# lonelycorn/mvSLAM

Hardware: AMD Instinct MI355X
Metric: image-pairs/sec (2k kp, 50k RANSAC hyp) (higher is better)
Workload: dtype f64; 1 GPU; 512 independent synthetic 640x480 pairs per GPU, 2000 keypoints (256-bit descriptors), 50000 8-point hypotheses per pair, full match+RANSAC+decompose+triangulate; pairs_per_gpu=512, keypoints=2000, hypotheses=50000, parallelism=pairs sharded, dp1, streams=2

## Files before the change

mvslam_amd/csrc/kernels.hip:

```cpp
#include <algorithm>
#include "kernels.hpp"

#include "device_math.hpp"
#include "match_fp4.hpp"
#include "prescreen.hpp"

namespace mvs {

constexpr uint32_t kKeyNone = 0xffffffffu;
__device__ __forceinline__ uint32_t bcnt_acc(uint32_t x, uint32_t acc)
{
    uint32_t r;
    asm("v_bcnt_u32_b32 %0, %1, %2" : "=v"(r) : "v"(x), "v"(acc));
    return r;
}
__device__ __forceinline__ void key_insert(uint32_t &k0, uint32_t &k1, uint32_t k)
{
    uint32_t m;
    asm("v_med3_u32 %0, %1, %2, %3" : "=v"(m) : "v"(k0), "v"(k1), "v"(k));
    k1 = m;
    k0 = min(k0, k);
}

constexpr int kTopkWaves = 16;
// ... 2425 lines not shown
                best = s_cnt[c];
                win = c;
            }
        s_win = win;
    }
    __syncthreads();
    const int win = s_win;
    if (win < 0) {
        clear_tail(0);
        return;
    }
    const double *src = b.cand_pts + ((size_t)pair * 4 + win) * b.max_kp * 3;
    const uint8_t *okw = okf + (size_t)win * b.max_kp;
    const uint16_t *inl = b.inl + base;
    const int n_pts = block_compact(
        n_inl, s_tot, [&](int j) { return okw[j] != 0; },
        [&](int j, int pos) {
            double *d = b.points + (base + pos) * 3;
            d[0] = src[j * 3]; d[1] = src[j * 3 + 1]; d[2] = src[j * 3 + 2];
            b.point_idx[base + pos] = inl[j];
        });
    clear_tail(n_pts);
    if (tid == 0) {
        const double *Rw = fm->R[win >> 1];
        const bool flip = (win & 1) != 0;
        const double t[3] = {flip ? -fm->T[0] : fm->T[0], flip ? -fm->T[1] : fm->T[1], flip ? -fm->T[2] : fm->T[2]};
        double Rr[3][3], RT[3][3];
#pragma unroll
        for (int i = 0; i < 3; ++i)
#pragma unroll
            for (int j = 0; j < 3; ++j) {
                Rr[i][j] = Rw[i * 3 + j];
                res->R1to2[i * 3 + j] = Rw[i * 3 + j];
            }
        rectify3(Rr);
#pragma unroll
        for (int i = 0; i < 3; ++i)
#pragma unroll
            for (int j = 0; j < 3; ++j)
                RT[i][j] = Rr[j][i];
        rectify3(RT);
#pragma unroll
        for (int i = 0; i < 3; ++i) {
            res->t1to2[i] = t[i];
            res->t[i] = -((RT[i][0] * t[0] + RT[i][1] * t[1]) + RT[i][2] * t[2]);
#pragma unroll
            for (int j = 0; j < 3; ++j)
                res->R[i * 3 + j] = RT[i][j];
        }
        res->n_points = n_pts;
        res->valid = 1;
    }
}

#ifdef MVS_DEBUG_HOOKS
#include "kernels_experiments.hip"
#endif

constexpr int kCntThreads = 768;
constexpr int kCntPpl = 2;
constexpr int kSolveBlock = 64;
#ifdef MVS_DEBUG_HOOKS
static int kSplitMinPairs = 3;
void set_split_min_pairs(int v) { kSplitMinPairs = v; }
#else
constexpr int kSplitMinPairs = 3;
#endif

static bool prescreened_launch(const BatchDev &b, int n_active, int H)
{
    const int cus = b.cu_count > 0 ? b.cu_count : 256;
    return n_active >= kSplitMinPairs || (kSplitMinPairs == 3 && n_active == 2 && 2 * ((H + kHypPerBlock - 1) / kHypPerBlock) > cus);
}

static size_t count_lds_bytes(int max_kp)
{
    const int bw = 64 * kCntPpl;
    return (size_t)((max_kp + bw - 1) / bw) * bw * 4 * sizeof(double);
}

bool kernel_desc(int id, int max_kp, int desc_words, KernelDesc *out)
{
    KernelDesc d{nullptr, nullptr, 0, 0};
    switch (id) {
    case kKMatchTopk:
        d.name = desc_words == 4 ? "match_topk_kernel<4>" : desc_words == 16 ? "match_topk_kernel<16>" : "match_mfma_kernel<true>";
        d.fn = desc_words == 4    ? reinterpret_cast<const void *>(match_topk_kernel<4>)
               : desc_words == 16 ? reinterpret_cast<const void *>(match_topk_kernel<16>)
                                  : reinterpret_cast<const void *>(match_mfma_kernel<true>);
        d.threads = desc_words == 8 ? kMmThreads : 1024;
        break;
    case kKMatchTopkVec:
        d.name = "match_topk_kernel<8>";
        d.fn = reinterpret_cast<const void *>(match_topk_kernel<8>);
        d.threads = 1024;
        break;
    case kKMatchCompact:
        d.name = "match_compact_kernel";
        d.fn = reinterpret_cast<const void *>(match_compact_kernel);
        d.threads = 1024;
        break;
    case kKRansacFused:
        d.name = "ransac_kernel<false, true, (mvs::Solve)2>";
        d.fn = reinterpret_cast<const void *>(ransac_kernel<false, true, Solve::GuardedCheap>);
        d.threads = kHypPerBlock;
        break;
    case kKRansacSolve:
        d.name = "ransac_solve_list_kernel";
        d.fn = reinterpret_cast<const void *>(ransac_solve_list_kernel);
        d.threads = kSolveBlock;
        break;
    case kKRansacSelect:
        d.name = "ransac_select_kernel";
        d.fn = reinterpret_cast<const void *>(ransac_select_kernel);
        d.threads = kSelThreads;
        d.dynamic_lds = (size_t)max_kp * 4 * sizeof(double);
        break;
    case kKPairPrepare:
        d.name = "pair_prepare_kernel";
        d.fn = reinterpret_cast<const void *>(pair_prepare_kernel);
        d.threads = 256;
        break;
    case kKRansacPrescreen:
        d.name = "ransac_prescreen_kernel";
        d.fn = reinterpret_cast<const void *>(ransac_prescreen_kernel);
        d.threads = 64;
        break;
    case kKRansacExactList:
        d.name = "ransac_exact_list_kernel";
        d.fn = reinterpret_cast<const void *>(ransac_exact_list_kernel);
        d.threads = 64;
        break;
    case kKRansacCount2:
        d.name = "ransac_count2_kernel<768, 2>";
        d.fn = reinterpret_cast<const void *>(ransac_count2_kernel<kCntThreads, kCntPpl>);
        d.threads = kCntThreads;
        d.dynamic_lds = count_lds_bytes(max_kp);
        break;
    case kKRansacCountPilot:
        d.name = "ransac_finish_mfma_kernel<false, true>";
        d.fn = reinterpret_cast<const void *>(ransac_finish_mfma_kernel<false, true>);
        d.threads = kFinishThreads;
        d.dynamic_lds = (size_t)kDenseChunk * 64;
        break;
    case kKRansacCountFinish:
        d.name = "ransac_finish_mfma_kernel<false, false>";
        d.fn = reinterpret_cast<const void *>(ransac_finish_mfma_kernel<false>);
        d.threads = kFinishThreads;
        d.dynamic_lds = (size_t)kDenseChunk * 64;
        break;
    case kKRansacCountFinishRest:
        d.name = "ransac_finish_upper_kernel<false>";
        d.fn = reinterpret_cast<const void *>(ransac_finish_upper_kernel<false>);
        d.threads = kFinUpperThreads;
        d.dynamic_lds = (size_t)kFinUpperChunk * 64 + (size_t)(kFinUpperThreads / 64) * kDenseWin * 16;
        break;
    case kKRansacCountMfma:
        d.name = "ransac_count_mfma_kernel<false, 512, 4, 672>";
        d.fn = reinterpret_cast<const void *>(ransac_count_mfma_kernel<false, kDenseThreads, kDenseBatches>);
        d.threads = kDenseThreads;
        d.dynamic_lds = (size_t)kDenseChunkD * 64 + (size_t)(kDenseThreads / 64) * kDenseWin * 16;
        break;
    case kKRansacSurvivors:
        d.name = "ransac_survivors_kernel";
        d.fn = reinterpret_cast<const void *>(ransac_survivors_kernel);
        d.threads = 256;
        break;
    case kKFinModel:
        d.name = "finalize_model_kernel";
        d.fn = reinterpret_cast<const void *>(finalize_model_kernel);
        d.threads = kFinThreads;
        break;
    case kKTriangulate:
        d.name = "triangulate_kernel";
        d.fn = reinterpret_cast<const void *>(triangulate_kernel);
        d.threads = 256;
        break;
    case kKFinSelect:
        d.name = "finalize_select_kernel";
        d.fn = reinterpret_cast<const void *>(finalize_select_kernel);
        d.threads = kFinThreads;
        break;
#ifdef MVS_DEBUG_HOOKS
    case kKRansacCount32:
        d.name = "ransac_count32_kernel<768, 4, 4, 1, false>";
        d.fn = reinterpret_cast<const void *>(ransac_count32_kernel<kCnt32Threads, kCnt32Ppl, kCnt32Slots, 1>);
        d.threads = kCnt32Threads;
        d.dynamic_lds = count32_lds_bytes(max_kp);
        break;
#endif
    default: return false;
    }
    *out = d;
    return true;
}

hipError_t prepare_kernels()
{
    const void *fns[] = {
#ifdef MVS_DEBUG_HOOKS
                         reinterpret_cast<const void *>(ransac_count32_kernel<kCnt32Threads, kCnt32Ppl, kCnt32Slots, 1>),
                         reinterpret_cast<const void *>(ransac_count32_kernel<kCnt32Threads, kCnt32Ppl, kCnt32Slots, 1, true>),
                         reinterpret_cast<const void *>(ransac_count32_kernel<kCnt32Threads, kCnt32Ppl, kCnt32Slots, 2>),
                         reinterpret_cast<const void *>(ransac_count32_kernel<kCnt32Threads, kCnt32Ppl, kCnt32Slots, 2, true>),
#endif
                         reinterpret_cast<const void *>(ransac_count2_kernel<kCntThreads, kCntPpl>),
                         reinterpret_cast<const void *>(ransac_count2_kernel<kCntThreads, kCntPpl, true>),
                         reinterpret_cast<const void *>(ransac_count_mfma_kernel<false, kDenseThreads, kDenseBatches>),
                         reinterpret_cast<const void *>(ransac_count_mfma_kernel<true, kDenseThreads, kDenseBatches>),
                         reinterpret_cast<const void *>(ransac_finish_mfma_kernel<false>),
                         reinterpret_cast<const void *>(ransac_finish_mfma_kernel<true>),
                         reinterpret_cast<const void *>(ransac_finish_mfma_kernel<false, true>),
                         reinterpret_cast<const void *>(ransac_finish_mfma_kernel<true, true>),
                         reinterpret_cast<const void *>(ransac_finish_upper_kernel<false>),
                         reinterpret_cast<const void *>(ransac_finish_upper_kernel<true>),
                         reinterpret_cast<const void *>(ransac_select_kernel)};
    for (const void *f : fns) {
        const hipError_t e = hipFuncSetAttribute(f, hipFuncAttributeMaxDynamicSharedMemorySize, kMaxKp * 32);
        if (e != hipSuccess)
            return e;
    }
    return hipSuccess;
}

#ifdef MVS_DEBUG_HOOKS
static int g_match_mfma = 1;
void set_match_mfma(int v) { g_match_mfma = v; }
#else
constexpr int g_match_mfma = 1;
#endif

void launch_match_topk(const BatchDev &b, const RunParams &rp, int n_active, hipStream_t stream, LaunchTimer *lt)
{
    const dim3 grid((b.max_kp + 63) / 64, n_active), block(1024);
    const double ratio = rp.ratio, md = rp.max_dist;
    const int mm_groups8 = ((b.max_kp + kMmQueries - 1) / kMmQueries) * n_active;
    const bool mfma8 = b.desc_words == 8 && (g_match_mfma == 2 || (g_match_mfma == 1 && mm_groups8 >= 512));
    if (lt) lt->mark(b.desc_words == 8 && !mfma8 ? kKMatchTopkVec : kKMatchTopk);
    switch (b.desc_words) {
    case 4: hipLaunchKernelGGL(match_topk_kernel<4>, grid, block, 0, stream, b, ratio, md); break;
    case 8: {
        if (mfma8) {
            const dim3 mgrid((b.max_kp + kMmQueries - 1) / kMmQueries, n_active);
            const int cap = match_cap_distance(ratio, md);
            if (cap >= 0)
                hipLaunchKernelGGL(match_mfma_kernel<true>, mgrid, dim3(kMmThreads), 0, stream, b, ratio, md, cap);
            else
                hipLaunchKernelGGL(match_mfma_kernel<false>, mgrid, dim3(kMmThreads), 0, stream, b, ratio, md, 0);
        } else
            hipLaunchKernelGGL(match_topk_kernel<8>, grid, block, 0, stream, b, ratio, md);
        break;
    }
    case 16: hipLaunchKernelGGL(match_topk_kernel<16>, grid, block, 0, stream, b, ratio, md); break;
    default: break;
    }
}

void launch_match_compact(const BatchDev &b, const RunParams &, int n_active, hipStream_t stream, LaunchTimer *lt)
{
    if (lt) lt->mark(kKMatchCompact);
    hipLaunchKernelGGL(match_compact_kernel, dim3(n_active), dim3(1024), 0, stream, b);
}

void launch_prep_points(const BatchDev &b, const double *uv1, const double *uv2, int n_active, hipStream_t stream)
{
    hipLaunchKernelGGL(prep_points_kernel, dim3((b.max_kp + 255) / 256, n_active), dim3(256), 0, stream, b, uv1, uv2);
}

#ifdef MVS_DEBUG_HOOKS
static int g_count_dense = 1;
static int g_dense_margin = kDenseMargin;
static int g_pilot_hyp = kPilotMfmaHyp;
void set_count_dense(int v)
{
    if (v >= 100000)
        g_pilot_hyp = v - 100000;
    else if (v >= 1000)
        g_dense_margin = v - 1000;
    else
        g_count_dense = v;
}
static int g_force_mode = -1;
void set_prescreen_force(int m) { g_force_mode = m; }
hipError_t prescreen_fallback_waves(unsigned int *out, bool reset)
{
    hipError_t e = hipMemcpyFromSymbol(out, HIP_SYMBOL(g_ps_fallback_waves), sizeof(*out));
    const unsigned int zero = 0;
    if (e == hipSuccess && reset)
        e = hipMemcpyToSymbol(HIP_SYMBOL(g_ps_fallback_waves), &zero, sizeof(zero));
    return e;
}

void launch_prescreen_only(const BatchDev &b, const RunParams &rp, int n_active, int mode, hipStream_t stream)
{
    hipLaunchKernelGGL(pair_prepare_kernel, dim3(n_active), dim3(256), 0, stream, b, rp, mode);
    hipLaunchKernelGGL(ransac_prescreen_kernel, dim3((rp.num_hypotheses + 63) / 64, n_active), dim3(64), 0, stream, b, rp);
}
#else
constexpr int g_dense_margin = kDenseMargin;
constexpr int g_pilot_hyp = kPilotMfmaHyp;
constexpr int g_force_mode = -1;
#endif

static void launch_counting(const BatchDev &b, const RunParams &rp, int n_active, hipStream_t stream, LaunchTimer *lt, bool stats,
                            hipEvent_t after_dense = nullptr)
{
    const int H = rp.num_hypotheses;
    const int n_groups4 = (H + kCntSlots - 1) / kCntSlots;
    const int wpw = kCntThreads / 64;
    int wg = (512 + n_active - 1) / n_active;
    wg = std::max(wg, 4);
    wg = std::min(wg, std::max(1, (n_groups4 + wpw - 1) / wpw));
    const size_t lds_cnt = count_lds_bytes(b.max_kp);
#ifdef MVS_DEBUG_HOOKS
    if (g_count_dense == 0) {
        if (lt) lt->mark(kKRansacCount32);
        launch_count32<1>(b, rp, wg, n_active, stats, stream);
    } else
#endif
    {
        if (lt) lt->mark(kKRansacCountPilot);
        const dim3 pilot_grid(n_active, (std::min(H, g_pilot_hyp) + kFinishThreads - 1) / kFinishThreads);
        if (stats)
            hipLaunchKernelGGL((ransac_finish_mfma_kernel<true, true>), pilot_grid, dim3(kFinishThreads), (size_t)kDenseChunk * 64,
                               stream, b, rp, 0);
        else
            hipLaunchKernelGGL((ransac_finish_mfma_kernel<false, true>), pilot_grid, dim3(kFinishThreads), (size_t)kDenseChunk * 64,
                               stream, b, rp, 0);
        if (lt) lt->mark(kKRansacCountMfma);
        const size_t lds_dense = (size_t)kDenseChunkD * 64 + (size_t)(kDenseThreads / 64) * kDenseWin * 16;
        const dim3 dense_grid(((H + kDenseThreads - 1) / kDenseThreads + kDenseBatches - 1) / kDenseBatches, n_active);
        if (stats)
            hipLaunchKernelGGL((ransac_count_mfma_kernel<true, kDenseThreads, kDenseBatches>), dense_grid, dim3(kDenseThreads),
                               lds_dense, stream, b, rp, g_dense_margin);
        else
            hipLaunchKernelGGL((ransac_count_mfma_kernel<false, kDenseThreads, kDenseBatches>), dense_grid, dim3(kDenseThreads),
                               lds_dense, stream, b, rp, g_dense_margin);
        if (after_dense) (void)hipEventRecord(after_dense, stream);
        if (lt) lt->mark(kKRansacCountFinish);
#ifdef MVS_DEBUG_HOOKS
        if (g_count_dense == 2) {
            launch_count32<2>(b, rp, wg, n_active, stats, stream);
        } else
#endif
        {
            hipLaunchKernelGGL(ransac_list_sort_kernel, dim3(n_active), dim3(kSortThreads), 0, stream, b);
            if (stats)
                hipLaunchKernelGGL(ransac_finish_mfma_kernel<true>, dim3(n_active, 1), dim3(kFinishThreads), (size_t)kDenseChunk * 64,
                                   stream, b, rp, 0);
            else
                hipLaunchKernelGGL(ransac_finish_mfma_kernel<false>, dim3(n_active, 1), dim3(kFinishThreads), (size_t)kDenseChunk * 64,
                                   stream, b, rp, 0);
            if ((H + kFinishThreads - 1) / kFinishThreads > 1) {
                const size_t lds_up = (size_t)kFinUpperChunk * 64 + (size_t)(kFinUpperThreads / 64) * kDenseWin * 16;
                if (lt) lt->mark(kKRansacCountFinishRest);
                if (stats)
                    hipLaunchKernelGGL(ransac_finish_upper_kernel<true>, dim3(n_active, kFinUpperWg), dim3(kFinUpperThreads), lds_up,
                                       stream, b, rp);
                else
                    hipLaunchKernelGGL(ransac_finish_upper_kernel<false>, dim3(n_active, kFinUpperWg), dim3(kFinUpperThreads), lds_up,
                                       stream, b, rp);
            }
        }
    }
    if (lt) lt->mark(kKRansacCount2);
    if (stats)
        hipLaunchKernelGGL((ransac_count2_kernel<kCntThreads, kCntPpl, true>), dim3(wg, n_active), dim3(kCntThreads), lds_cnt,
                           stream, b, rp, wg);
    else
        hipLaunchKernelGGL((ransac_count2_kernel<kCntThreads, kCntPpl>), dim3(wg, n_active), dim3(kCntThreads), lds_cnt, stream,
                           b, rp, wg);
}

static void launch_prescreened(const BatchDev &b, const RunParams &rp, int n_active, hipStream_t stream, LaunchTimer *lt,
                               bool stats, hipEvent_t after_dense = nullptr)
{
    const int H = rp.num_hypotheses;
    const int G = (H + kHypPerBlock - 1) / kHypPerBlock;
    if (lt) lt->mark(kKPairPrepare);
    hipLaunchKernelGGL(pair_prepare_kernel, dim3(n_active), dim3(256), 0, stream, b, rp, g_force_mode);
    if (lt) lt->mark(kKRansacPrescreen);
    hipLaunchKernelGGL(ransac_prescreen_kernel, dim3((H + 63) / 64, n_active), dim3(64), 0, stream, b, rp);
    if (lt) lt->mark(kKRansacSolve);
    hipLaunchKernelGGL(mode0_list_kernel, dim3(1), dim3(256), 0, stream, b, n_active);
    static_assert(kSolveBlock == 64, "ransac_solve_list_kernel takes blocks of 64 hypotheses");
    hipLaunchKernelGGL(ransac_solve_list_kernel, dim3(2048), dim3(64), 0, stream, b, rp,
                       G * (kHypPerBlock / kSolveBlock));
    launch_counting(b, rp, n_active, stream, lt, stats, after_dense);
    if (lt) lt->mark(kKRansacSurvivors);
    hipLaunchKernelGGL(ransac_survivors_kernel, dim3(kSurvWg, n_active), dim3(256), 0, stream, b, rp, n_active);
    if (lt) lt->mark(kKRansacExactList);
    hipLaunchKernelGGL(ransac_exact_list_kernel, dim3(1024), dim3(64), 0, stream, b, rp, 0);
    if (lt) lt->mark(kKRansacSelect);
    hipLaunchKernelGGL(ransac_select_kernel, dim3(n_active), dim3(kSelThreads), (size_t)b.max_kp * 4 * sizeof(double), stream,
                       b, rp, 1);
}

void launch_ransac(const BatchDev &b, const RunParams &rp, int n_active, bool stats, hipStream_t stream, LaunchTimer *lt,
                   hipEvent_t after_dense)
{
    const int G = (rp.num_hypotheses + kHypPerBlock - 1) / kHypPerBlock;
    const dim3 grid(G, n_active), block(kHypPerBlock);
    const bool split_ok = !stats && b.hyp_F && prescreened_launch(b, n_active, rp.num_hypotheses);
    if (!split_ok || b.hyp_count) {
        if (lt) lt->mark(kKRansacFused);
        if (!stats)
            hipLaunchKernelGGL((ransac_kernel<false, true, Solve::GuardedCheap>), grid, block, 0, stream, b, rp);
        else
            hipLaunchKernelGGL((ransac_kernel<true, true, Solve::Guarded>), grid, block, 0, stream, b, rp);
        if (stats && b.hyp_F && !b.hyp_count && prescreened_launch(b, n_active, rp.num_hypotheses))
            launch_prescreened(b, rp, n_active, stream, nullptr, true);
    } else {
        launch_prescreened(b, rp, n_active, stream, lt, false, after_dense);
    }
}

void launch_finalize(const BatchDev &b, const RunParams &rp, int n_active, int mode, hipStream_t stream, LaunchTimer *lt)
{
    if (lt) lt->mark(kKFinModel);
    hipLaunchKernelGGL(finalize_model_kernel, dim3(n_active), dim3(kFinThreads), 0, stream, b, rp, mode);
    if (lt) lt->mark(kKTriangulate);
    hipLaunchKernelGGL(triangulate_kernel, dim3((b.max_kp + 255) / 256, n_active), dim3(256), 0, stream, b);
    if (lt) lt->mark(kKFinSelect);
    hipLaunchKernelGGL(finalize_select_kernel, dim3(n_active), dim3(kFinThreads), 0, stream, b);
}

#ifdef MVS_DEBUG_HOOKS
#include "kernels_audit.hip"
#endif


__global__ __launch_bounds__(256) void single_params_kernel(BatchDev b, SingleParams sp, const uint4 *in)
{
    const int t = blockIdx.x * 256 + threadIdx.x;
    if (t == 0) {
        const_cast<int32_t *>(b.n1)[0] = sp.n1;
        const_cast<int32_t *>(b.n2)[0] = sp.n2;
        const_cast<int64_t *>(b.gidx)[0] = sp.gidx;
    }
    if (t < 9) {
        const_cast<double *>(b.K)[t] = sp.K[t];
        const_cast<double *>(b.Kinv)[t] = sp.Kinv[t];
    }
    if (in) {
        uint4 *dst[4] = {reinterpret_cast<uint4 *>(const_cast<uint32_t *>(b.desc1)), reinterpret_cast<uint4 *>(const_cast<uint32_t *>(b.desc2)),
                         reinterpret_cast<uint4 *>(const_cast<float *>(b.kp1)), reinterpret_cast<uint4 *>(const_cast<float *>(b.kp2))};
        size_t off = 0;
#pragma unroll
        for (int k = 0; k < 4; ++k) {
            const size_t n16 = sp.part_bytes[k] / 16;
            for (size_t i = t; i < n16; i += (size_t)gridDim.x * 256)
                dst[k][i] = in[off + i];
            if (t == 0 && (sp.part_bytes[k] & 8u))
                reinterpret_cast<uint2 *>(dst[k] + n16)[0] = reinterpret_cast<const uint2 *>(in + off + n16)[0];
            off += (sp.part_bytes[k] + 15) / 16;
        }
    }
}
void launch_single_params(const BatchDev &b, const SingleParams &sp, const void *in, hipStream_t stream)
{
    hipLaunchKernelGGL(single_params_kernel, dim3(in ? 32 : 1), dim3(256), 0, stream, b, sp, reinterpret_cast<const uint4 *>(in));
}
__global__ __launch_bounds__(256) void single_gather_kernel(BatchDev b, int rows, int flags, unsigned char *out)
{
    const SingleLayout L = single_layout(rows, flags);
    const int tid = blockIdx.x * 256 + threadIdx.x, nth = gridDim.x * 256;
    const uint32_t *r32 = reinterpret_cast<const uint32_t *>(b.results);
    for (int i = tid; i < (int)(sizeof(mvs_pair_result) / 4); i += nth)
        reinterpret_cast<uint32_t *>(out)[i] = r32[i];
    if (flags & 1)
        for (int i = tid; i < rows; i += nth)
            out[L.mask + i] = b.mask[i];
    if (flags & 2)
        for (int i = tid; i < rows * 3; i += nth)
            reinterpret_cast<double *>(out + L.points)[i] = b.points[i];
    if (flags & 4)
        for (int i = tid; i < rows; i += nth)
            reinterpret_cast<int32_t *>(out + L.idx)[i] = b.point_idx[i];
    if (flags & 8)
        for (int i = tid; i < rows; i += nth)
            reinterpret_cast<mvs_match *>(out + L.matches)[i] = b.matches[i];
}
void launch_single_gather(const BatchDev &b, int rows, int flags, unsigned char *out, hipStream_t stream)
{
    hipLaunchKernelGGL(single_gather_kernel, dim3(16), dim3(256), 0, stream, b, rows, flags, out);
}

void launch_fundamental(const double *p1, const double *p2, double *F, int *ok, hipStream_t stream)
{
    hipLaunchKernelGGL(fundamental_kernel, dim3(1), dim3(64), 0, stream, p1, p2, F, ok);
}

}
```

mvslam_amd/csrc/kernels_audit.hip:

```cpp
#ifndef MVS_DEBUG_HOOKS
#error "kernels_audit.hip belongs to the diagnostics build"
#endif

__global__ __launch_bounds__(256) void pairstep_check_kernel(const double *rows, int n, unsigned long long *out)
{
    const int i = blockIdx.x * 256 + threadIdx.x;
    if (i >= n)
        return;
    double A[2][2][3], V[2][2][3], W[2][2];
#pragma unroll
    for (int v = 0; v < 2; ++v) {
#pragma unroll
        for (int r = 0; r < 2; ++r) {
            double sd = 0.0;
#pragma unroll
            for (int k = 0; k < 3; ++k) {
                A[v][r][k] = rows[(size_t)i * 6 + r * 3 + k];
                V[v][r][k] = r == k ? 1.0 : 0.0;
                sd = dfma(A[v][r][k], A[v][r][k], sd);
            }
            W[v][r] = sd;
        }
    }
    {
        const double g2 = dfma(W[0][0], W[0][0], W[0][1] * W[0][1]) + 0x1p-300;
        double h;
        const double gamma = sqrt_fast_nz_h(g2, h);
        const double e = dabs(dfma(-gamma, h + h, 1.0));
        atomicMax(&out[3], (unsigned long long)__double_as_longlong(e));
    }
    bool ch0 = false, ch1 = false, bad0 = false, bad1 = false;
    unsigned r0 = 0, r1 = 0;
    double q0 = 0x1p1000, q1 = 0x1p1000;
    jacobi_pair<3, 3, true, true, true>(A[0][0], A[0][1], V[0][0], V[0][1], W[0][0], W[0][1], ch0, r0, bad0, q0);
    jacobi_pair<3, 3, false, false, false>(A[1][0], A[1][1], V[1][0], V[1][1], W[1][0], W[1][1], ch1, r1, bad1, q1);
    if (ch0 != ch1) {
        atomicAdd(&out[2], 1ull);
        return;
    }
    if (!ch0 || !(q0 >= kGuardQMin) || !(W[1][0] + W[1][1] <= kGuardWSumMax))
        return;
    atomicAdd(&out[1], 1ull);
    bool same = __double_as_longlong(W[0][0]) == __double_as_longlong(W[1][0]) &&
                __double_as_longlong(W[0][1]) == __double_as_longlong(W[1][1]);
#pragma unroll
    for (int r = 0; r < 2; ++r)
#pragma unroll
        for (int k = 0; k < 3; ++k)
            same = same && __double_as_longlong(A[0][r][k]) == __double_as_longlong(A[1][r][k]) &&
                   __double_as_longlong(V[0][r][k]) == __double_as_longlong(V[1][r][k]);
    if (!same)
        atomicAdd(&out[0], 1ull);
}

void launch_pairstep_check(const double *rows, int n, unsigned long long *out, hipStream_t stream)
{
    hipLaunchKernelGGL(pairstep_check_kernel, dim3((n + 255) / 256), dim3(256), 0, stream, rows, n, out);
}

void launch_fastmath_check(const double *x, const double *y, int n, unsigned long long *out, hipStream_t stream)
{
    hipLaunchKernelGGL(fastmath_check_kernel, dim3((n + 255) / 256), dim3(256), 0, stream, x, y, n, out);
}


template <int PHASE>
__global__ __launch_bounds__(256, 1) void audit_kernel(BatchDev b, RunParams rp, unsigned long long *out, int32_t *maxc)
{
    extern __shared__ __attribute__((aligned(16))) double s_apts[];
    const int pair = blockIdx.y, g = blockIdx.x, tid = threadIdx.x, lane = tid & 63;
    const int M = min(b.M[pair], b.max_kp);
    if (M < 8)
        return;
    const int H = rp.num_hypotheses;
    const uint32_t h = (uint32_t)g * kHypPerBlock + tid;
    const bool live = h < (uint32_t)H;
    const uint32_t hh = live ? h : (uint32_t)(H - 1);
    const uint64_t seed = rp.seed + (uint64_t)b.gidx[pair];
    const double *P = b.pts + (size_t)pair * b.max_kp * 4;
    {
        const double2 *src = reinterpret_cast<const double2 *>(P);
        double2 *dst = reinterpret_cast<double2 *>(s_apts);
        for (int i = tid; i < 2 * M; i += kHypPerBlock)
            dst[i] = src[i];
        __syncthreads();
    }
    double F[9];
    unsigned rot = 0, pairs = 0;
    bool bad = false;
    bool ok = solve_hypothesis<Solve::GuardedCheap>(seed, hh, M, rp.sampler, P, F, rot, pairs, bad);
    if (__builtin_expect(__any(bad), 0)) {
        rot = 0;
        pairs = 0;
        ok = solve_hypothesis<Solve::Ieee>(seed, hh, M, rp.sampler, P, F, rot, pairs, bad);
    }
    const unsigned sweeps = pairs / 36u;
    const double thr = pair_max_error_sq(b, rp, pair);
    const int mode = b.mode[pair];
    const size_t Hp = (size_t)b.max_groups * kHypPerBlock;
    const size_t rec = (size_t)pair * Hp + h;
    const int state = live ? (int)b.hyp_okf[rec] : kPsInvalid;
    const double4 *L4 = reinterpret_cast<const double4 *>(s_apts);
    unsigned long long v_state = 0, v_count = 0, v_upper = 0, v_lower = 0, v_band = 0, n_cert = 0, v_F = 0, v_surv = 0, n_nan = 0,
                       v_m0 = 0, n_match = 0;
    double worst = 0.0;
    int cJ = 0;
    if (PHASE == 0) {
        if (live && mode != 0) {
            if (state == kPsInvalid && ok) ++v_state;
            if (state == kPsApprox && !ok) ++v_state;
            if (state == kPsApprox) {
                ++n_cert;
                const double *Fo = b.hyp_F + rec * kHypRec;
                int U = 0, L = 0;
                if (mode == 1) {
                    const float *fo = b.hyp_r32 + rec * kHypRec32;
                    float Ft[9];
#pragma unroll
                    for (int k = 0; k < 9; ++k)
                        Ft[k] = fo[k];
                    const float tu = fo[9], tl = fo[10];
                    const double beta = (double)tu - thr;
                    for (int i = 0; i < M; ++i) {
                        const double4 p = L4[i];
                        const double rJ = epipolar_residual(F, p.x, p.y, p.z, p.w);
                        const float x1 = (float)p.x, y1 = (float)p.y, x2 = (float)p.z, y2 = (float)p.w;
                        const float u0 = __builtin_fmaf(x2, Ft[0], __builtin_fmaf(y2, Ft[3], Ft[6]));
                        const float u1 = __builtin_fmaf(x2, Ft[1], __builtin_fmaf(y2, Ft[4], Ft[7]));
                        const float u2 = __builtin_fmaf(x2, Ft[2], __builtin_fmaf(y2, Ft[5], Ft[8]));
                        const float r32 = __builtin_fabsf(__builtin_fmaf(u0, x1, __builtin_fmaf(u1, y1, u2)));
                        cJ += rJ < thr ? 1 : 0;
                        U += r32 < tu ? 1 : 0;
                        L += r32 < tl ? 1 : 0;
                        if (rJ != rJ) {
                            ++n_nan;
                        } else {
                            const double d = dabs(rJ - (double)r32);
                            ++n_match;
                            if (!(d <= beta)) ++v_band;
                            worst = fmax(worst, d / beta);
                        }
                    }
                } else {
                    double Ft[9];
#pragma unroll
                    for (int k = 0; k < 9; ++k)
                        Ft[k] = Fo[k];
                    const double tu = Fo[9];
                    const double beta = tu - thr;
                    const double tl = thr - (tu - thr) * (1.0 + 1e-9) - 1e-15 * thr;
                    for (int i = 0; i < M; ++i) {
                        const double4 p = L4[i];
                        const double rJ = epipolar_residual(F, p.x, p.y, p.z, p.w);
                        const double rt = epipolar_residual(Ft, p.x, p.y, p.z, p.w);
                        cJ += rJ < thr ? 1 : 0;
                        U += rt < tu ? 1 : 0;
                        L += rt < tl ? 1 : 0;
                        if (rJ != rJ) {
                            ++n_nan;
                        } else {
                            const double d = dabs(rJ - rt);
                            ++n_match;
                            if (!(d <= beta)) ++v_band;
                            worst = fmax(worst, d / beta);
                        }
                    }
                }
                if (U < cJ) ++v_upper;
                if (L > cJ) ++v_lower;
            }
        }
    } else {
        for (int i = 0; i < M; ++i) {
            const double4 p = L4[i];
            const double rJ = epipolar_residual(F, p.x, p.y, p.z, p.w);
            cJ += rJ < thr ? 1 : 0;
        }
        if (live) {
            const int cnt = b.hyp_cnt[rec];
            const int bound = b.bound[pair];
            const double *Fo = b.hyp_F + rec * kHypRec;
            const bool counted = cnt >= 0 && cnt != 0x7fffffff;
            if ((state == kPsInvalid) != !ok) ++v_state;
            if (state == kPsNeedExact) ++v_state;
            if (state == kPsExact) {
                bool same = true;
#pragma unroll
                for (int k = 0; k < 9; ++k)
                    same = same && __double_as_longlong(Fo[k]) == __double_as_longlong(F[k]);
                if (!same) ++v_F;
            }
            if (mode == 0) {
                if (ok && counted && cnt != cJ) ++v_m0;
                if (ok && !counted && !(cJ < bound)) ++v_count;
                if (ok && counted && cnt < bound && !(cJ < bound)) ++v_count;
            } else {
                if (state == kPsApprox) {
                    if (cnt >= bound) ++v_surv;
                    if (!(cJ < bound)) ++v_count;
                } else if (state == kPsExact && counted) {
                    ++n_cert;
                    if (cnt < cJ) ++v_upper;
                }
            }
        }
    }
    auto wsum = [&](unsigned long long v) {
#pragma unroll
        for (int o = 32; o > 0; o >>= 1)
            v += __shfl_xor(v, o);
        return v;
    };
    const unsigned long long vals[16] = {live ? 1ull : 0ull, v_state, v_count, v_upper, v_lower, v_band, 0ull, n_cert, 0ull, v_F,
                                         v_surv, n_nan, v_m0, n_match, (live && !ok) ? 1ull : 0ull, live ? sweeps : 0u};
#pragma unroll
    for (int k = 0; k < 16; ++k) {
        if (k == 6 || k == 8)
            continue;
        const unsigned long long t = wsum(vals[k]);
        if (lane == 0 && t)
            atomicAdd(&out[k], t);
    }
    unsigned sw = live ? sweeps : 0u;
    int mc = (live && ok) ? cJ : -1;
#pragma unroll
    for (int o = 32; o > 0; o >>= 1) {
        sw = max(sw, (unsigned)__shfl_xor((int)sw, o));
        mc = max(mc, __shfl_xor(mc, o));
        worst = fmax(worst, __shfl_xor(worst, o));
    }
    if (lane == 0) {
        atomicMax(&out[8], (unsigned long long)sw);
        atomicMax(&out[6], (unsigned long long)__double_as_longlong(worst));
        if (PHASE == 1)
            atomicMax(&maxc[pair], mc);
    }
}

__global__ __launch_bounds__(256) void keep_only_kernel(BatchDev b, const int32_t *keep)
{
    const int pair = blockIdx.y;
    const size_t Hp = (size_t)b.max_groups * kHypPerBlock;
    const size_t h = (size_t)blockIdx.x * 256 + threadIdx.x;
    const int k = keep[pair];
    if (h < Hp && k >= 0 && h != (size_t)k)
        b.hyp_okf[(size_t)pair * Hp + h] = (uint8_t)kPsInvalid;
}
void launch_count_only(const BatchDev &b, const RunParams &rp, int n_active, int pmode, int dense, const int32_t *keep,
                       hipStream_t stream)
{
    launch_prescreen_only(b, rp, n_active, pmode, stream);
    if (keep)
        hipLaunchKernelGGL(keep_only_kernel, dim3(b.max_groups, n_active), dim3(256), 0, stream, b, keep);
    const int old = g_count_dense;
    g_count_dense = dense;
    launch_counting(b, rp, n_active, stream, nullptr, false);
    g_count_dense = old;
}
__global__ __launch_bounds__(64) void indicator_probe_kernel(const float *a, const float *tu, const float *tl, const float *T,
                                                             int n, float *ind_u, float *ind_l, float *scale)
{
    const int i = blockIdx.x * 64 + threadIdx.x;
    if (i >= n)
        return;
    const f32x2 negH = {-0x1p100f, -0x1p100f};
    bool lpos;
    const float t2u = dense_t2_upper(tu[i], T[i], true), t2l = dense_t2_lower(tl[i], T[i], true, lpos);
    const f32x2 x = {a[i], -a[i]};
    const f32x2 sq = pk_mul(x, x);
    const f32x2 u = pk_ind(sq, negH, f32x2{t2u, t2u}), l = pk_ind(sq, negH, f32x2{t2l, t2l});
    ind_u[i] = u.x == u.y ? u.x : -1.f;
    ind_l[i] = l.x == l.y ? l.x : -1.f;
    scale[i] = dense_scale(tu[i], T[i], true);
}
void launch_indicator_probe(const float *a, const float *tu, const float *tl, const float *T, int n, float *ind_u, float *ind_l,
                            float *scale, hipStream_t stream)
{
    hipLaunchKernelGGL(indicator_probe_kernel, dim3((n + 63) / 64), dim3(64), 0, stream, a, tu, tl, T, n, ind_u, ind_l, scale);
}
__global__ __launch_bounds__(64) void rounding_probe_kernel(const double *in, int n, double *out)
{
    const int i = blockIdx.x * 64 + threadIdx.x;
    if (i >= n)
        return;
    const double *q = in + (size_t)i * 19;
    double Fn[9], Fn3[3][3], Fa[9], Fb[9];
#pragma unroll
    for (int k = 0; k < 9; ++k) {
        Fn[k] = q[k];
        Fn3[k / 3][k % 3] = q[k];
    }
    EightNorm nm;
    nm.s1 = q[9]; nm.s2 = q[10]; nm.m1x = q[11]; nm.m1y = q[12]; nm.m2x = q[13]; nm.m2y = q[14];
    prescreen_denormalise(Fn, nm, Fa);
    denormalise_exact(Fn3, nm, Fb);
    out[2 * i] = epipolar_residual(Fa, q[15], q[16], q[17], q[18]);
    out[2 * i + 1] = epipolar_residual(Fb, q[15], q[16], q[17], q[18]);
}
void launch_rounding_probe(const double *in, int n, double *out, hipStream_t stream)
{
    hipLaunchKernelGGL(rounding_probe_kernel, dim3((n + 63) / 64), dim3(64), 0, stream, in, n, out);
}

hipError_t launch_audit(const BatchDev &b, const RunParams &rp, int n_active, int phase, unsigned long long *out, int32_t *maxc,
                        hipStream_t stream)
{
    const int G = (rp.num_hypotheses + kHypPerBlock - 1) / kHypPerBlock;
    const size_t lds = (size_t)b.max_kp * 4 * sizeof(double);
    const void *fn = phase == 0 ? reinterpret_cast<const void *>(audit_kernel<0>) : reinterpret_cast<const void *>(audit_kernel<1>);
    const hipError_t e = hipFuncSetAttribute(fn, hipFuncAttributeMaxDynamicSharedMemorySize, kMaxKp * 32);
    if (e != hipSuccess)
        return e;
    if (phase == 0)
        hipLaunchKernelGGL(audit_kernel<0>, dim3(G, n_active), dim3(kHypPerBlock), lds, stream, b, rp, out, maxc);
    else
        hipLaunchKernelGGL(audit_kernel<1>, dim3(G, n_active), dim3(kHypPerBlock), lds, stream, b, rp, out, maxc);
    return hipGetLastError();
}
```

Before: 126,600 pairs/s.

## Move dense/finish counting ahead of the solve-list kernels in prescreened path

Splits the counting launcher into dense, finish and double-precision stages and reorders the prescreened pipeline so the MFMA dense counting and finish stages run right after prescreen, before mode0_list and ransac_solve_list. The after_dense event is now recorded earlier, so work waiting on it on the other stream can start sooner and overlap. This relies on the dense/finish kernels not depending on the solve-list outputs. If they do, results could be wrong.

```diff
diff --git a/mvslam_amd/csrc/kernels.hip b/mvslam_amd/csrc/kernels.hip
--- a/mvslam_amd/csrc/kernels.hip
+++ b/mvslam_amd/csrc/kernels.hip
@@ -2751,67 +2751,82 @@
 constexpr int g_force_mode = -1;
 #endif
 
-static void launch_counting(const BatchDev &b, const RunParams &rp, int n_active, hipStream_t stream, LaunchTimer *lt, bool stats,
-                            hipEvent_t after_dense = nullptr)
-{
-    const int H = rp.num_hypotheses;
-    const int n_groups4 = (H + kCntSlots - 1) / kCntSlots;
+static int counting_wg(const RunParams &rp, int n_active)
+{
+    const int n_groups4 = (rp.num_hypotheses + kCntSlots - 1) / kCntSlots;
     const int wpw = kCntThreads / 64;
     int wg = (512 + n_active - 1) / n_active;
     wg = std::max(wg, 4);
-    wg = std::min(wg, std::max(1, (n_groups4 + wpw - 1) / wpw));
-    const size_t lds_cnt = count_lds_bytes(b.max_kp);
+    return std::min(wg, std::max(1, (n_groups4 + wpw - 1) / wpw));
+}
+
+static void launch_counting_dense(const BatchDev &b, const RunParams &rp, int n_active, hipStream_t stream, LaunchTimer *lt, bool stats)
+{
+    const int H = rp.num_hypotheses;
 #ifdef MVS_DEBUG_HOOKS
     if (g_count_dense == 0) {
         if (lt) lt->mark(kKRansacCount32);
-        launch_count32<1>(b, rp, wg, n_active, stats, stream);
+        launch_count32<1>(b, rp, counting_wg(rp, n_active), n_active, stats, stream);
+        return;
+    }
+#endif
+    if (lt) lt->mark(kKRansacCountPilot);
+    const dim3 pilot_grid(n_active, (std::min(H, g_pilot_hyp) + kFinishThreads - 1) / kFinishThreads);
+    if (stats)
+        hipLaunchKernelGGL((ransac_finish_mfma_kernel<true, true>), pilot_grid, dim3(kFinishThreads), (size_t)kDenseChunk * 64,
+                           stream, b, rp, 0);
+    else
+        hipLaunchKernelGGL((ransac_finish_mfma_kernel<false, true>), pilot_grid, dim3(kFinishThreads), (size_t)kDenseChunk * 64,
+                           stream, b, rp, 0);
+    if (lt) lt->mark(kKRansacCountMfma);
+    const size_t lds_dense = (size_t)kDenseChunkD * 64 + (size_t)(kDenseThreads / 64) * kDenseWin * 16;
+    const dim3 dense_grid(((H + kDenseThreads - 1) / kDenseThreads + kDenseBatches - 1) / kDenseBatches, n_active);
+    if (stats)
+        hipLaunchKernelGGL((ransac_count_mfma_kernel<true, kDenseThreads, kDenseBatches>), dense_grid, dim3(kDenseThreads),
+                           lds_dense, stream, b, rp, g_dense_margin);
+    else
+        hipLaunchKernelGGL((ransac_count_mfma_kernel<false, kDenseThreads, kDenseBatches>), dense_grid, dim3(kDenseThreads),
+                           lds_dense, stream, b, rp, g_dense_margin);
+}
+
+static void launch_counting_finish(const BatchDev &b, const RunParams &rp, int n_active, hipStream_t stream, LaunchTimer *lt, bool stats)
+{
+    const int H = rp.num_hypotheses;
+#ifdef MVS_DEBUG_HOOKS
+    if (g_count_dense == 0)
+        return;
+#endif
+    if (lt) lt->mark(kKRansacCountFinish);
+#ifdef MVS_DEBUG_HOOKS
+    if (g_count_dense == 2) {
+        launch_count32<2>(b, rp, counting_wg(rp, n_active), n_active, stats, stream);
     } else
 #endif
     {
-        if (lt) lt->mark(kKRansacCountPilot);
-        const dim3 pilot_grid(n_active, (std::min(H, g_pilot_hyp) + kFinishThreads - 1) / kFinishThreads);
+        hipLaunchKernelGGL(ransac_list_sort_kernel, dim3(n_active), dim3(kSortThreads), 0, stream, b);
         if (stats)
-            hipLaunchKernelGGL((ransac_finish_mfma_kernel<true, true>), pilot_grid, dim3(kFinishThreads), (size_t)kDenseChunk * 64,
+            hipLaunchKernelGGL(ransac_finish_mfma_kernel<true>, dim3(n_active, 1), dim3(kFinishThreads), (size_t)kDenseChunk * 64,
                                stream, b, rp, 0);
         else
-            hipLaunchKernelGGL((ransac_finish_mfma_kernel<false, true>), pilot_grid, dim3(kFinishThreads), (size_t)kDenseChunk * 64,
+            hipLaunchKernelGGL(ransac_finish_mfma_kernel<false>, dim3(n_active, 1), dim3(kFinishThreads), (size_t)kDenseChunk * 64,
                                stream, b, rp, 0);
-        if (lt) lt->mark(kKRansacCountMfma);
-        const size_t lds_dense = (size_t)kDenseChunkD * 64 + (size_t)(kDenseThreads / 64) * kDenseWin * 16;
-        const dim3 dense_grid(((H + kDenseThreads - 1) / kDenseThreads + kDenseBatches - 1) / kDenseBatches, n_active);
-        if (stats)
-            hipLaunchKernelGGL((ransac_count_mfma_kernel<true, kDenseThreads, kDenseBatches>), dense_grid, dim3(kDenseThreads),
-                               lds_dense, stream, b, rp, g_dense_margin);
-        else
-            hipLaunchKernelGGL((ransac_count_mfma_kernel<false, kDenseThreads, kDenseBatches>), dense_grid, dim3(kDenseThreads),
-                               lds_dense, stream, b, rp, g_dense_margin);
-        if (after_dense) (void)hipEventRecord(after_dense, stream);
-        if (lt) lt->mark(kKRansacCountFinish);
-#ifdef MVS_DEBUG_HOOKS
-        if (g_count_dense == 2) {
-            launch_count32<2>(b, rp, wg, n_active, stats, stream);
-        } else
-#endif
-        {
-            hipLaunchKernelGGL(ransac_list_sort_kernel, dim3(n_active), dim3(kSortThreads), 0, stream, b);
+        if ((H + kFinishThreads - 1) / kFinishThreads > 1) {
+            const size_t lds_up = (size_t)kFinUpperChunk * 64 + (size_t)(kFinUpperThreads / 64) * kDenseWin * 16;
+            if (lt) lt->mark(kKRansacCountFinishRest);
             if (stats)
-                hipLaunchKernelGGL(ransac_finish_mfma_kernel<true>, dim3(n_active, 1), dim3(kFinishThreads), (size_t)kDenseChunk * 64,
-                                   stream, b, rp, 0);
+                hipLaunchKernelGGL(ransac_finish_upper_kernel<true>, dim3(n_active, kFinUpperWg), dim3(kFinUpperThreads), lds_up,
+                                   stream, b, rp);
             else
-                hipLaunchKernelGGL(ransac_finish_mfma_kernel<false>, dim3(n_active, 1), dim3(kFinishThreads), (size_t)kDenseChunk * 64,
-                                   stream, b, rp, 0);
-            if ((H + kFinishThreads - 1) / kFinishThreads > 1) {
-                const size_t lds_up = (size_t)kFinUpperChunk * 64 + (size_t)(kFinUpperThreads / 64) * kDenseWin * 16;
-                if (lt) lt->mark(kKRansacCountFinishRest);
-                if (stats)
-                    hipLaunchKernelGGL(ransac_finish_upper_kernel<true>, dim3(n_active, kFinUpperWg), dim3(kFinUpperThreads), lds_up,
-                                       stream, b, rp);
-                else
-                    hipLaunchKernelGGL(ransac_finish_upper_kernel<false>, dim3(n_active, kFinUpperWg), dim3(kFinUpperThreads), lds_up,
-                                       stream, b, rp);
-            }
-        }
-    }
+                hipLaunchKernelGGL(ransac_finish_upper_kernel<false>, dim3(n_active, kFinUpperWg), dim3(kFinUpperThreads), lds_up,
+                                   stream, b, rp);
+        }
+    }
+}
+
+static void launch_counting_double(const BatchDev &b, const RunParams &rp, int n_active, hipStream_t stream, LaunchTimer *lt, bool stats)
+{
+    const int wg = counting_wg(rp, n_active);
+    const size_t lds_cnt = count_lds_bytes(b.max_kp);
     if (lt) lt->mark(kKRansacCount2);
     if (stats)
         hipLaunchKernelGGL((ransac_count2_kernel<kCntThreads, kCntPpl, true>), dim3(wg, n_active), dim3(kCntThreads), lds_cnt,
@@ -2830,12 +2845,15 @@
     hipLaunchKernelGGL(pair_prepare_kernel, dim3(n_active), dim3(256), 0, stream, b, rp, g_force_mode);
     if (lt) lt->mark(kKRansacPrescreen);
     hipLaunchKernelGGL(ransac_prescreen_kernel, dim3((H + 63) / 64, n_active), dim3(64), 0, stream, b, rp);
+    launch_counting_dense(b, rp, n_active, stream, lt, stats);
+    if (after_dense) (void)hipEventRecord(after_dense, stream);
+    launch_counting_finish(b, rp, n_active, stream, lt, stats);
     if (lt) lt->mark(kKRansacSolve);
     hipLaunchKernelGGL(mode0_list_kernel, dim3(1), dim3(256), 0, stream, b, n_active);
     static_assert(kSolveBlock == 64, "ransac_solve_list_kernel takes blocks of 64 hypotheses");
     hipLaunchKernelGGL(ransac_solve_list_kernel, dim3(2048), dim3(64), 0, stream, b, rp,
                        G * (kHypPerBlock / kSolveBlock));
-    launch_counting(b, rp, n_active, stream, lt, stats, after_dense);
+    launch_counting_double(b, rp, n_active, stream, lt, stats);
     if (lt) lt->mark(kKRansacSurvivors);
     hipLaunchKernelGGL(ransac_survivors_kernel, dim3(kSurvWg, n_active), dim3(256), 0, stream, b, rp, n_active);
     if (lt) lt->mark(kKRansacExactList);
diff --git a/mvslam_amd/csrc/kernels_audit.hip b/mvslam_amd/csrc/kernels_audit.hip
--- a/mvslam_amd/csrc/kernels_audit.hip
+++ b/mvslam_amd/csrc/kernels_audit.hip
@@ -254,7 +254,9 @@
         hipLaunchKernelGGL(keep_only_kernel, dim3(b.max_groups, n_active), dim3(256), 0, stream, b, keep);
     const int old = g_count_dense;
     g_count_dense = dense;
-    launch_counting(b, rp, n_active, stream, nullptr, false);
+    launch_counting_dense(b, rp, n_active, stream, nullptr, false);
+    launch_counting_finish(b, rp, n_active, stream, nullptr, false);
+    launch_counting_double(b, rp, n_active, stream, nullptr, false);
     g_count_dense = old;
 }
 __global__ __launch_bounds__(64) void indicator_probe_kernel(const float *a, const float *tu, const float *tl, const float *T,
```

Result: no change. 126,000 pairs/s (-0.5%).
